# polixir/emei

Measured on AMD Instinct MI355X. Metric: env-steps/s, higher is better.
Workload: dtype f64

## Files before the change

### emei_amd/_lib.py

```python
import ctypes as C
import os

_HERE = os.path.dirname(os.path.abspath(__file__))
LIB_PATH = os.environ.get("EMEI_HIP_LIB") or os.path.join(_HERE, "libemei_hip.so")

ENV_IDS = {
    "CartPoleSwingUp": 0,
    "CartPoleBalancing": 1,
    "ReboundInvertedPendulumBalancing": 2,
    "BoundaryInvertedPendulumBalancing": 3,
    "ReboundInvertedPendulumSwingUp": 4,
    "BoundaryInvertedPendulumSwingUp": 5,
    "HalfCheetahRunning": 6,
    "ReboundInvertedDoublePendulumBalancing": 7,
    "BoundaryInvertedDoublePendulumBalancing": 8,
    "ReboundInvertedDoublePendulumSwingUp": 9,
    "BoundaryInvertedDoublePendulumSwingUp": 10,
    "HopperRunning": 11,
}
PRECISION_REF, PRECISION_F32 = 0, 1
ACT_U8, ACT_I32, ACT_I64, ACT_F32 = 0, 1, 2, 3
FLAG_AUTO_RESET = 1
DONE_TERMINAL, DONE_TRUNCATED = 1, 2
OK, ERR_INVALID, ERR_HIP, ERR_UNSUPPORTED, ERR_STATE = 0, -1, -2, -3, -4
# ... 47 lines not shown
        ("solver", C.c_uint32),
        ("env_params", C.c_double * MAX_ENV_PARAMS),
        ("ode_method", C.c_int32),
        ("rollout_chunk_steps", C.c_int32),
    ]


_vp, _i32, _i64, _u32, _u64, _dbl = C.c_void_p, C.c_int32, C.c_int64, C.c_uint32, C.c_uint64, C.c_double
SYMBOLS = {
    "emei_create": (C.c_int, [C.POINTER(EmeiConfig), C.POINTER(_vp)]),
    "emei_destroy": (C.c_int, [_vp]),
    "emei_last_error": (C.c_char_p, []),
    "emei_abi_version": (C.c_int, []),
    "emei_model_constants": (C.c_int, [C.c_int, _vp, C.c_int]),
    "emei_model_invweights": (C.c_int, [C.c_int, _vp, C.c_int]),
    "emei_env_dims": (C.c_int, [C.c_int, C.POINTER(C.c_int), C.POINTER(C.c_int), C.POINTER(C.c_int)]),
    "emei_reset": (C.c_int, [_vp, _u64, _vp]),
    "emei_set_seed": (C.c_int, [_vp, _u64]),
    "emei_get_solver_cap_hits": (C.c_int, [_vp, _vp, _vp]),
    "emei_get_rollout_faults": (C.c_int, [_vp, _vp, _vp]),
    "emei_last_rollout_kernel": (C.c_int, [_vp]),
    "emei_set_obs_peers": (C.c_int, [_vp, C.c_int, C.POINTER(_vp), _i64, _i64, _i32]),
    "emei_peer_buffer_create": (C.c_int, [C.c_int, _u64, C.POINTER(_vp), _vp]),
    "emei_peer_buffer_open": (C.c_int, [C.c_int, _vp, C.POINTER(_vp)]),
    "emei_peer_buffer_close": (C.c_int, [C.c_int, _vp]),
    "emei_peer_buffer_destroy": (C.c_int, [C.c_int, _vp]),
    "emei_set_state": (C.c_int, [_vp, _vp, C.c_int, _vp]),
    "emei_get_state": (C.c_int, [_vp, _vp, _vp]),
    "emei_get_obs": (C.c_int, [_vp, _vp, _vp]),
    "emei_freeze": (C.c_int, [_vp, _vp]),
# ... 82 lines not shown
```

### emei_amd/csrc/abi.hip

```cpp
#include <hip/hip_runtime.h>

#include <cmath>
#include <cstdarg>
#include <cstdio>
#include <cstring>
#include <ctime>
#include <new>

#include "launch.h"
#include "body_kernels.h"
#include "cheetah_model.h"
#include "hopper_model.h"
#include "dpend_model.h"

using namespace emei;

struct emei_env {
    emei_config cfg;
    int obs_dim, act_dim, state_dim;
    size_t real_size;
    void* state;
    int32_t* steps;
    uint32_t* episode;
    unsigned long long* done_mask;
// ... 64 lines not shown
        case EMEI_IP_REBOUND_SWINGUP:
        case EMEI_IP_BOUNDARY_SWINGUP: n = ip_xml_constants(buf); break;
        case EMEI_IDP_REBOUND_BALANCING:
        case EMEI_IDP_BOUNDARY_BALANCING:
        case EMEI_IDP_REBOUND_SWINGUP:
        case EMEI_IDP_BOUNDARY_SWINGUP: n = dpend::xml_constants(buf); break;
        case EMEI_HALFCHEETAH_RUNNING: n = cheetah::xml_constants(buf); break;
        case EMEI_HOPPER_RUNNING: n = hopper::xml_constants(buf); break;
        case EMEI_CARTPOLE_SWINGUP:
        case EMEI_CARTPOLE_BALANCING: return fail(EMEI_ERR_UNSUPPORTED, "emei_model_constants: CartPole has no model file (cartpole.py:22-27)");
        default: return fail(EMEI_ERR_INVALID, "unknown env_id %d", env_id);
    }
    if (n > capacity) return fail(EMEI_ERR_INVALID, "emei_model_constants: %d values, capacity %d", n, capacity);
    memcpy(out, buf, n * sizeof(double));
    return n;
}

extern "C" EMEI_API int emei_model_invweights(int env_id, double* out, int capacity) {
    if (!out || capacity < 0) return fail(EMEI_ERR_INVALID, "emei_model_invweights: bad argument");
    double buf[32];
    int n;
    switch (env_id) {
        case EMEI_IP_REBOUND_BALANCING:
        case EMEI_IP_BOUNDARY_BALANCING:
        case EMEI_IP_REBOUND_SWINGUP:
        case EMEI_IP_BOUNDARY_SWINGUP: {
            constexpr IpModel m = ip_make_model(false);
            buf[0] = m.invw, buf[1] = m.invw_hinge, n = 2;
            break;
        }
// ... 1158 lines not shown
```

### emei_amd/csrc/body_kernels.h

```cpp
#pragma once
#include "emei_device.h"
#include "launch.h"

namespace emei {

struct EnvParams {
    uint32_t mask = 0;
    double v[EMEI_MAX_ENV_PARAMS] = {0};
    double get(int k, double dflt) const { return (mask >> k) & 1u ? v[k] : dflt; }
};

struct NoiseSpec {
    float init[EMEI_MAX_STATE_DIM] = {0}, obs[EMEI_MAX_STATE_DIM] = {0};
    int32_t shared = 0;
};
template <int NS>
struct NoiseArgs {
    float init[NS], obs[NS];
    int32_t shared, obs_on;
    NoiseArgs() = default;
    explicit NoiseArgs(const NoiseSpec& h) : shared(h.shared), obs_on(0) {
        for (int i = 0; i < NS; ++i) init[i] = h.init[i], obs[i] = h.obs[i], obs_on |= h.obs[i] != 0.f;
    }
};
// ... 19 lines not shown
        boxmuller(r.v[0], r.v[1], z[4 * b], z[4 * b + 1]);
        boxmuller(r.v[2], r.v[3], z[4 * b + 2], z[4 * b + 3]);
    }
#pragma unroll
    for (int i = 0; i < NS; ++i) {
        const R d = (R)__fmul_rn(sig[i], z[i]);
        s[i] = ASSIGN ? d : s[i] + d;
    }
}
template <class Body>
__device__ __forceinline__ void body_init(typename Body::real (&s)[Body::NS], uint64_t seed, uint64_t env, uint32_t episode,
                                          const NoiseArgs<Body::NS>& ns) {
    gauss_state<typename Body::real, Body::NS, true>(s, seed, env, episode, 0u, ns.init, ns.shared != 0);
    Body::init_base(s);
}

template <class Body, bool RK4>
__device__ __forceinline__ void body_substep(typename Body::real (&s)[Body::NS], const typename Body::real (&ctrl)[Body::NA],
                                             const typename Body::Model& m, bool semi, const TrigCtx& trig,
                                             typename Body::Warm& warm) {
    using R = typename Body::real;
    constexpr int NV = Body::NS / 2;
    const R dt = (R)m.dt;
    R q[NV], v[NV], acc[NV];
#pragma unroll
    for (int i = 0; i < NV; ++i) q[i] = s[i], v[i] = s[NV + i];
    if constexpr (!RK4) {
        typename Body::Warm cold{};
        Body::accel(q, v, ctrl, m, dt, acc, trig, cold);
#pragma unroll
// ... 161 lines not shown
    constexpr int kWaves = kBlock / kWave;
    constexpr int kActVec = (kWave * NA + 3) / 4, kObsVec = (kWave * NO + 3) / 4;
    constexpr int kActIt = (kActVec + kWave - 1) / kWave, kObsIt = (kObsVec + kWave - 1) / kWave;
    __shared__ __attribute__((aligned(16))) float act_s[kWaves][kActIt * kWave * 4];
    __shared__ __attribute__((aligned(16))) float obs_s[kWaves][kObsIt * kWave * 4];
    __shared__ SinCosEntry trig_s[kTrigTableSize];
    stage_trig_table<kBlock>(trig_s, a.trig);
    TrigCtx trig;
    trig.tab = trig_s;
    __shared__ R scratch_s[(Body::kScratchPerLane > 0 ? Body::kScratchPerLane : 1) * (Body::kScratchPerLane > 0 ? kBlock : 1)];
    if constexpr (Body::kScratchPerLane > 0) trig.scratch = scratch_s;
    trig.scratch_stride = kBlock;
    trig.cap_hits = a.cap_hits;
    EMEI_PROFILE_BEGIN();
    const int lane = threadIdx.x & (kWave - 1), wv = threadIdx.x / kWave;
    constexpr bool kQueue = QUEUE;
    uint32_t ticket = 0;
    [[maybe_unused]] bool first_item = true;
    if constexpr (kQueue) {
        if (lane == 0) ticket = __hip_atomic_fetch_add(a.work + WorkQueue::kTicket, 1u, __ATOMIC_RELAXED, __HIP_MEMORY_SCOPE_AGENT);
    }
#pragma nounroll
    for (;;) {
    EMEI_CLOCK_BEGIN();
    uint32_t blk = blockIdx.x, chunk = 0;
    int t_begin = 0, t_end = a.n_steps;
    if constexpr (kQueue) {
        ticket = __builtin_amdgcn_readfirstlane(ticket);
        if (ticket >= a.n_items) {
            EMEI_CLOCK_WORKER_EXIT();
// ... 78 lines not shown
        } else {
#pragma unroll
            for (int c = 0; c < kActIt; ++c) ((float4*)act_s[wv])[c * kWave + lane] = av[c];
            wave_lds_fence();
#pragma unroll
            for (int k = 0; k < NA; ++k) ctrl[k] = (R)act_s[wv][lane * NA + k];
            wave_lds_fence();
            if (t + 1 < t_end) fetch_actions(t + 1);
        }

        R pre[NS];
#pragma unroll
        for (int k = 0; k < NS; ++k) pre[k] = s[k];
        typename Body::Warm warm{};
        for (int k = 0; k < a.freq_rate; ++k) {
            body_substep<Body, RK4>(s, ctrl, a.m, a.semi != 0, trig, warm);
            if (obs_noise)
                gauss_state<R, NS, false>(s, a.seed ^ kObsNoiseKey, a.env_offset + (uint64_t)i, episode,
                                          ((uint32_t)steps * (uint32_t)a.freq_rate + (uint32_t)k) * (uint32_t)((NS + 3) / 4),
                                          a.noise.obs, a.noise.shared != 0);
        }
        EMEI_MARK(step_io);
        float o[NO];
        R rew;
        bool term;
        Body::outputs(s, pre, ctrl, a.m, a.freq_rate, o, rew, term, trig);
        ++steps;
        const bool trunc = (a.max_episode_steps > 0) & (steps >= a.max_episode_steps);
        done = active ? ((term ? EMEI_DONE_TERMINAL : 0u) | (trunc ? EMEI_DONE_TRUNCATED : 0u)) : 0u;

        if (a.obs_out) {
            float* mine = &obs_s[wv][lane * NO];
#pragma unroll
            for (int k = 0; k < NO; ++k) mine[k] = o[k];
            wave_lds_fence();
            float* dst = a.obs_out + ((int64_t)t * n + i0) * NO;
            if (wave_envs == kWave && (((uintptr_t)dst) & 15u) == 0) {
#pragma unroll
                for (int c = 0; c < kObsIt; ++c) {
                    const int vec = c * kWave + lane;
                    if (vec < kObsVec) store_body_out<Body::kStreamOutputs>((float4*)dst + vec, ((const float4*)obs_s[wv])[vec]);
// ... 133 lines not shown
        __syncthreads();
    }
    if (threadIdx.x == 0) *out = part[0];
}
template <class Body, typename T>
__global__ void __launch_bounds__(kBlock)
    body_terminal_kernel(const T* obs, uint8_t* terminal, int64_t n, typename Body::Model m) {
    const int64_t i = (int64_t)blockIdx.x * kBlock + threadIdx.x;
    if (i >= n) return;
    terminal[i] = (uint8_t)Body::batch_terminal(obs + i * Body::NO, m);
}

template <class Body, bool RK4, typename T>
__global__ void __launch_bounds__(kBlock)
    body_next_obs_kernel(const T* obs, const float* actions, T* next_obs, int64_t n, int freq_rate, int semi,
                         typename Body::Model m, const SinCosEntry* trig_tab) {
    using R = typename Body::real;
    constexpr int NS = Body::NS, NO = Body::NO, NA = Body::NA;
    static_assert(NS == NO, "observation and state must have the same layout");
    __shared__ SinCosEntry trig_s[kTrigTableSize];
    stage_trig_table(trig_s, trig_tab);
    TrigCtx trig;
    trig.tab = trig_s;
    __shared__ R scratch_s[(Body::kScratchPerLane > 0 ? Body::kScratchPerLane : 1) * (Body::kScratchPerLane > 0 ? kBlock : 1)];
    if constexpr (Body::kScratchPerLane > 0) trig.scratch = scratch_s;
    const int64_t i = (int64_t)blockIdx.x * kBlock + threadIdx.x;
    if (i >= n) return;
    R s[NS], pre[NS], ctrl[NA], rew;
#pragma unroll
    for (int k = 0; k < NS; ++k) s[k] = pre[k] = (R)obs[i * NO + k];
#pragma unroll
    for (int k = 0; k < NA; ++k) ctrl[k] = (R)actions[i * NA + k];
    typename Body::Warm warm{};
    for (int k = 0; k < freq_rate; ++k) body_substep<Body, RK4>(s, ctrl, m, semi != 0, trig, warm);
    if constexpr (sizeof(T) == 8) {
        double o[NO];
        Body::obs_of(s, o, m);
#pragma unroll
        for (int k = 0; k < NO; ++k) next_obs[i * NO + k] = o[k];
    } else {
        float o[NO];
        bool term;
        Body::outputs(s, pre, ctrl, m, freq_rate, o, rew, term, trig);
#pragma unroll
        for (int k = 0; k < NO; ++k) next_obs[i * NO + k] = o[k];
    }
}

template <class Body, bool RK4, bool DRAWN = false, bool KEEP = false, class Spec = CandidateSpec>
__global__ void __launch_bounds__(kBlock)
    body_plan_kernel(const typename Body::real* state, const double* start_rows, const float* actions, int64_t n_envs,
                     int32_t n_cand, int32_t horizon, double discount, int freq_rate, int semi, typename Body::Model m,
                     const SinCosEntry* trig_tab, unsigned long long* cap_hits, double* ret_out, int32_t* len_out, float* final_obs,
                     Spec sp, PlanPartial* partials) {
    using R = typename Body::real;
    constexpr int NS = Body::NS, NO = Body::NO, NA = Body::NA;
    __shared__ SinCosEntry trig_s[kTrigTableSize];
    stage_trig_table(trig_s, trig_tab);
    TrigCtx trig;
    trig.tab = trig_s;
    __shared__ R scratch_s[(Body::kScratchPerLane > 0 ? Body::kScratchPerLane : 1) * (Body::kScratchPerLane > 0 ? kBlock : 1)];
    if constexpr (Body::kScratchPerLane > 0) trig.scratch = scratch_s;
    trig.scratch_stride = kBlock;
    trig.cap_hits = cap_hits;
    const int64_t nk = n_envs * n_cand;
    const int64_t j = (int64_t)blockIdx.x * kBlock + threadIdx.x;
    const bool active = j < nk;
    const int64_t i = (active ? j : 0) / n_cand;
    R s[NS], parked[NS];
    if (start_rows) {
#pragma unroll
        for (int k = 0; k < NS; ++k) s[k] = (R)start_rows[i * NS + k];
    } else {
#pragma unroll
        for (int k = 0; k < NS; ++k) s[k] = state[(int64_t)k * n_envs + i];
    }
    Body::park(parked);
#pragma unroll
    for (int k = 0; k < NS; ++k) s[k] = active ? s[k] : parked[k];
// ... 230 lines not shown
```

### emei_amd/csrc/body_mpc_kernels.h

```cpp
#pragma once

namespace emei {

template <class Body>
struct BodyMpcArgs {
    typename Body::real* state;
    int32_t* steps;
    uint32_t* episode;
    const SinCosEntry* trig;
    unsigned long long* cap_hits;
    float* nominal;
    double* work;
    float* actions_out;
    float* obs_out;
    float* reward_out;
    uint8_t* done_out;
    double* plan_return_out;
    double* ess_out;
    double* elite_return_out;
    int64_t n;
    int32_t n_steps, horizon, n_cand, n_elites, iterations, freq_rate, max_episode_steps, semi;
    uint32_t flags;
    uint64_t reset_seed, env_offset, seed;
    double discount, temperature;
    float sigma, sigma_min, lo, hi, refill, nominal_lo, nominal_hi;
    NoiseArgs<Body::NS> noise;
    typename Body::Model m;
};

template <class Body, bool RK4, class Spec>
__device__ __forceinline__ void body_mpc_score(const typename Body::real (&s)[Body::NS], const Spec& sp, uint64_t g, int lane,
                                               const BodyMpcArgs<Body>& a, const TrigCtx& trig, double* wt, double& rs, int32_t& ks) {
    using R = typename Body::real;
    constexpr int NS = Body::NS, NO = Body::NO, NA = Body::NA;
    rs = __builtin_nan("");
    ks = INT32_MAX;
    for (int32_t k0 = 0; k0 < a.n_cand; k0 += kWave) {
        const int32_t k = k0 + lane;
        R cs[NS];
#pragma unroll
        for (int q = 0; q < NS; ++q) cs[q] = s[q];
        double ret = 0.0, gd = 1.0;
        bool live = k < a.n_cand;
        for (int32_t h = 0; h < a.horizon; ++h) {
            R ctrl[NA];
            CandidateWords cw(sp.seed, g, (uint32_t)k);
#pragma unroll
            for (int q = 0; q < NA; ++q) ctrl[q] = (R)draw_action(cw, sp, 1, 0, h, q, NA);
            R pre[NS];
#pragma unroll
            for (int q = 0; q < NS; ++q) pre[q] = cs[q];
            typename Body::Warm warm{};
            for (int f = 0; f < a.freq_rate; ++f) body_substep<Body, RK4>(cs, ctrl, a.m, a.semi != 0, trig, warm);
            float o[NO];
            R rew;
            bool term;
            Body::outputs(cs, pre, ctrl, a.m, a.freq_rate, o, rew, term, trig);
            if (live) {
                ret = ret + gd * (double)(float)rew;
                gd = gd * a.discount;
                if (term) live = false;
            }
            if (__ballot(live) == 0ull) break;
        }
        if (k < a.n_cand) {
            wt[k] = ret;
            if (plan_replaces(rs, ks, ret, k)) rs = ret, ks = k;
        }
    }
#pragma unroll
    for (int d = 1; d < kWave; d <<= 1) {
        const double r2 = __shfl_xor(rs, d, kWave);
        const int32_t k2 = __shfl_xor(ks, d, kWave);
        if (plan_replaces(rs, ks, r2, k2)) rs = r2, ks = k2;
    }
}

template <class Body, bool RK4>
__device__ __forceinline__ uint32_t body_mpc_act_step(typename Body::real (&s)[Body::NS], int32_t& steps, uint32_t& episode, float* nom,
                                                      int32_t n_comp, int32_t t, int64_t i, uint64_t g, int lane,
                                                      const BodyMpcArgs<Body>& a, const TrigCtx& trig) {
    using R = typename Body::real;
    constexpr int NS = Body::NS, NO = Body::NO, NA = Body::NA;
    const int64_t at = (int64_t)t * a.n + i;
    R ctrl[NA];
#pragma unroll
    for (int q = 0; q < NA; ++q) {
        const float av = nom[q];
        ctrl[q] = (R)av;
        if (lane == 0) a.actions_out[at * NA + q] = av;
    }
    R pre[NS];
#pragma unroll
    for (int q = 0; q < NS; ++q) pre[q] = s[q];
    typename Body::Warm warm{};
    for (int f = 0; f < a.freq_rate; ++f) body_substep<Body, RK4>(s, ctrl, a.m, a.semi != 0, trig, warm);
    float o[NO];
    R rew;
    bool term;
    Body::outputs(s, pre, ctrl, a.m, a.freq_rate, o, rew, term, trig);
    ++steps;
    const bool trunc = (a.max_episode_steps > 0) & (steps >= a.max_episode_steps);
    const uint32_t done = (term ? EMEI_DONE_TERMINAL : 0u) | (trunc ? EMEI_DONE_TRUNCATED : 0u);
    if (lane == 0) {
        if (a.obs_out) {
#pragma unroll
            for (int q = 0; q < NO; ++q) a.obs_out[at * NO + q] = o[q];
        }
        if (a.reward_out) a.reward_out[at] = (float)rew;
        if (a.done_out) a.done_out[at] = (uint8_t)done;
    }
    const bool reset_now = (a.flags & EMEI_FLAG_AUTO_RESET) != 0 && __builtin_amdgcn_readfirstlane(done) != 0u;
    if (reset_now) {
        ++episode;
        steps = 0;
// ... 25 lines not shown
}

template <class Body, bool RK4>
__global__ void __launch_bounds__(kBlock) body_mpc_mppi_kernel(const BodyMpcArgs<Body> a) {
    static_assert(Body::kFusedMpc && Body::kScratchPerLane == 0, "a body without block scratch that opted in");
    using R = typename Body::real;
    constexpr int kWavesPerBlock = kBlock / kWave;
    constexpr int NS = Body::NS, na = Body::NA;
    __shared__ SinCosEntry trig_s[kTrigTableSize];
    __shared__ float nom_s[kWavesPerBlock][EMEI_MPC_MAX_HORIZON * na];
    stage_trig_table(trig_s, a.trig);
    TrigCtx trig;
    trig.tab = trig_s;
    trig.scratch_stride = kBlock;
    trig.cap_hits = a.cap_hits;
    const int lane = (int)(threadIdx.x & (kWave - 1));
    const int wv = __builtin_amdgcn_readfirstlane((int)(threadIdx.x / kWave));
    const int64_t i = (int64_t)blockIdx.x * kWavesPerBlock + wv;
    if (i >= a.n) return;
    const int64_t n = a.n;
    const int32_t n_cand = a.n_cand;
    const int32_t n_comp = a.horizon * na;
    float* nom = nom_s[wv];
    for (int32_t c = lane; c < n_comp; c += kWave) nom[c] = a.nominal[((int64_t)(c / na) * n + i) * na + c % na];

    R s[NS];
#pragma unroll
    for (int k = 0; k < NS; ++k) s[k] = a.state[(int64_t)k * n + i];
    int32_t steps = a.steps[i];
    uint32_t episode = a.episode[i];
    const uint64_t g = a.env_offset + (uint64_t)i;
    double* wt = a.work + i * n_cand;
    CandidateSpecLds sp;
    sp.env_offset = a.env_offset;
    sp.nominal.p = (const __attribute__((address_space(3))) float*)nom;
    sp.sigma = a.sigma, sp.lo = a.lo, sp.hi = a.hi;
    uint32_t done = 0;

    for (int32_t t = 0; t < a.n_steps; ++t) {
        for (int32_t cc = lane; cc < n_comp; cc += kWave) nom[cc] = fminf(fmaxf(nom[cc], a.nominal_lo), a.nominal_hi);
        wave_lds_fence();
        sp.seed = a.seed + (uint64_t)t;
        double rs;
        int32_t ks;
        body_mpc_score<Body, RK4>(s, sp, g, lane, a, trig, wt, rs, ks);
        double z = 0.0, z2 = 0.0;
        for (int32_t k = lane; k < n_cand; k += kWave) {
            const double r = wt[k];
            const double e = exp((r - rs) / a.temperature);
            const double w = rs != rs ? 1.0 : (r != r ? 0.0 : (r == rs ? 1.0 : e));
            wt[k] = w;
            z += w, z2 += w * w;
        }
#pragma unroll
        for (int d = 1; d < kWave; d <<= 1) z += __shfl_xor(z, d, kWave);
#pragma unroll
        for (int d = 1; d < kWave; d <<= 1) z2 += __shfl_xor(z2, d, kWave);
        if (lane == 0) {
            if (a.plan_return_out) a.plan_return_out[(int64_t)t * n + i] = rs;
            if (a.ess_out) a.ess_out[(int64_t)t * n + i] = z * z / z2;
// ... 13 lines not shown
#pragma unroll
            for (int u = 0; u < 4; ++u) {
#pragma unroll
                for (int d = 1; d < kWave; d <<= 1) acc[u] += __shfl_xor(acc[u], d, kWave);
            }
            wave_lds_fence();
            if (lane == 0) {
#pragma unroll
                for (int u = 0; u < 4; ++u) {
                    const int32_t cc = c0 + u;
                    if (cc < n_comp) nom[cc] = (float)(acc[u] / z);
                }
            }
        }
        wave_lds_fence();
        done = body_mpc_act_step<Body, RK4>(s, steps, episode, nom, n_comp, t, i, g, lane, a, trig);
    }
    body_mpc_write_back<Body>(s, steps, episode, done, nom, n_comp, i, lane, wt, a);
}

template <class Body, bool RK4>
__global__ void __launch_bounds__(kBlock) body_mpc_cem_kernel(const BodyMpcArgs<Body> a) {
    static_assert(Body::kFusedMpc && Body::kScratchPerLane == 0, "a body without block scratch that opted in");
    using R = typename Body::real;
    constexpr int kWavesPerBlock = kBlock / kWave;
    constexpr int NS = Body::NS, na = Body::NA;
    __shared__ SinCosEntry trig_s[kTrigTableSize];
    __shared__ float nom_s[kWavesPerBlock][EMEI_MPC_MAX_HORIZON * na];
    __shared__ float sig_s[kWavesPerBlock][EMEI_MPC_MAX_HORIZON * na];
    __shared__ uint32_t hist_s[kWavesPerBlock][256];
    stage_trig_table(trig_s, a.trig);
    TrigCtx trig;
    trig.tab = trig_s;
    trig.scratch_stride = kBlock;
    trig.cap_hits = a.cap_hits;
    const int lane = (int)(threadIdx.x & (kWave - 1));
    const int wv = __builtin_amdgcn_readfirstlane((int)(threadIdx.x / kWave));
    const int64_t i = (int64_t)blockIdx.x * kWavesPerBlock + wv;
    if (i >= a.n) return;
    const int64_t n = a.n;
    const int32_t n_cand = a.n_cand;
    const int32_t n_comp = a.horizon * na;
    float* nom = nom_s[wv];
    float* sig = sig_s[wv];
    uint32_t* hist = hist_s[wv];
    for (int32_t c = lane; c < n_comp; c += kWave) nom[c] = a.nominal[((int64_t)(c / na) * n + i) * na + c % na];

    R s[NS];
#pragma unroll
    for (int k = 0; k < NS; ++k) s[k] = a.state[(int64_t)k * n + i];
// ... 7 lines not shown
    sp.sigma_map.p = (const __attribute__((address_space(3))) float*)sig;
    sp.lo = a.lo, sp.hi = a.hi;
    const double m_el = (double)a.n_elites;
    uint32_t done = 0;

    for (int32_t t = 0; t < a.n_steps; ++t) {
        for (int32_t it = 0; it < a.iterations; ++it) {
            for (int32_t cc = lane; cc < n_comp; cc += kWave) {
                nom[cc] = fminf(fmaxf(nom[cc], a.nominal_lo), a.nominal_hi);
                if (it == 0) sig[cc] = a.sigma;
            }
            wave_lds_fence();
            sp.seed = a.seed + (uint64_t)t * (uint64_t)a.iterations + (uint64_t)it;
            double rs;
            int32_t ks;
            body_mpc_score<Body, RK4>(s, sp, g, lane, a, trig, wt, rs, ks);
            const bool last_it = it == a.iterations - 1;
            if (lane == 0 && last_it && a.plan_return_out) a.plan_return_out[(int64_t)t * n + i] = rs;
            uint64_t prefix = 0ull;
            int32_t need = a.n_elites;
            for (int shift = 56; shift >= 0; shift -= 8) {
#pragma unroll
                for (int b = 0; b < 4; ++b) hist[4 * lane + b] = 0u;
                wave_lds_fence();
                for (int32_t k = lane; k < n_cand; k += kWave) {
                    const uint64_t key = plan_key(wt[k]);
                    const uint64_t high = shift == 56 ? 0ull : key >> (shift + 8);
                    if (high == prefix) atomicAdd(&hist[(uint32_t)(key >> shift) & 255u], 1u);
                }
                wave_lds_fence();
                int32_t cb[4], own = 0;
// ... 63 lines not shown
                if (lane == 0) {
#pragma unroll
                    for (int u = 0; u < 4; ++u) {
                        const int32_t cc = c0 + u;
                        if (cc >= n_comp) continue;
                        const double mu = s1[u] / m_el;
                        nom[cc] = (float)(m0[u] + mu);
                        sig[cc] = (float)sqrt(fmax(s2[u] / m_el - mu * mu, 0.0));
                    }
                }
            }
            wave_lds_fence();
            for (int32_t cc = lane; cc < n_comp; cc += kWave) sig[cc] = fmaxf(sig[cc], a.sigma_min);
            wave_lds_fence();
        }
        done = body_mpc_act_step<Body, RK4>(s, steps, episode, nom, n_comp, t, i, g, lane, a, trig);
    }
    body_mpc_write_back<Body>(s, steps, episode, done, nom, n_comp, i, lane, wt, a);
}

template <class Body>
static int launch_body_mpc(const BodyLaunch& L, const typename Body::Model& m) {
    const MpcLaunch& M = L.mpc;
    const bool cem = L.op == BODY_OP_MPC_CEM;
    if (M.horizon < 1 || M.horizon > EMEI_MPC_MAX_HORIZON) return EMEI_ERR_INVALID;
    if (cem && (M.iterations < 1 || M.n_elites < 1 || M.n_elites > L.plan.n_candidates)) return EMEI_ERR_INVALID;
    if (NoiseArgs<Body::NS>(L.noise).obs_on) return EMEI_ERR_UNSUPPORTED;
    BodyMpcArgs<Body> a;
    a.state = (typename Body::real*)L.state, a.steps = L.steps, a.episode = L.episode;
    a.trig = (const SinCosEntry*)L.trig, a.cap_hits = L.cap_hits;
    a.nominal = M.nominal, a.work = L.plan.return_out, a.actions_out = M.actions_out;
// ... 26 lines not shown
```

### emei_amd/csrc/dpend_model.h

```cpp
#pragma once
#include <cmath>
#include <cstring>

#include "emei_device.h"

namespace emei {
namespace dpend {

struct Model {
    double s1z, s2z, diag1, diag2, L1, mtot;
    double gx, gz, gear, x_lo, x_hi, margin, invw;
    double K, B, dmin, dmax, width;
    double dt, phi_off;
};

namespace host {
inline double capsule_mass(double rho, double r, double half) { return rho * (M_PI * r * r * 2 * half + 4.0 / 3.0 * M_PI * r * r * r); }
inline double capsule_inertia_perp(double rho, double r, double half) {
    double h = 2 * half, mcyl = rho * M_PI * r * r * h, msph = rho * 4.0 / 3.0 * M_PI * r * r * r;
    return mcyl * (3 * r * r + h * h) / 12 + msph * (2 * r * r / 5 + h * h / 4 + 3 * h * r / 8);
}
}

struct Xml {
    double rho, cart_r, cart_half, pole_r, pole_half, L1, gx, gz, gear, ctrl_lo, ctrl_hi, x_lo, x_hi, margin, solref_tc, dmin, dmax, width;
};
constexpr Xml kXml = {1000.0, 0.1, 0.1,
                      0.045, 0.3, 0.6,
                      1e-5, 9.81,
                      500.0, -1.0, 1.0,
                      -3.0, 3.0, 0.01,
                      0.02, 0.9, 0.95, 0.001};

inline Model make_model(bool swingup, double dt) {
    Model m;
    memset(&m, 0, sizeof(m));
    const double rho = kXml.rho;
    const double mc = host::capsule_mass(rho, kXml.cart_r, kXml.cart_half);
    const double mp = host::capsule_mass(rho, kXml.pole_r, kXml.pole_half);
    const double Ip = host::capsule_inertia_perp(rho, kXml.pole_r, kXml.pole_half);
    const double lc = kXml.pole_half, L1 = kXml.L1;
    m.s1z = mp * lc + mp * L1, m.s2z = mp * lc;
    m.diag1 = Ip + mp * lc * lc + mp * L1 * L1, m.diag2 = Ip + mp * lc * lc;
    m.L1 = L1, m.mtot = mc + 2 * mp;
    m.gx = kXml.gx, m.gz = kXml.gz;
    m.gear = kXml.gear;
    m.x_lo = kXml.x_lo, m.x_hi = kXml.x_hi, m.margin = kXml.margin;
    const double a = m.mtot, b = m.s1z, c = m.s2z, d = m.diag1, e = L1 * m.s2z, f = m.diag2;
    const double det = a * (d * f - e * e) - b * (b * f - e * c) + c * (b * e - d * c);
    m.invw = (d * f - e * e) / det;
    const double tc = kXml.solref_tc < 2 * dt ? 2 * dt : kXml.solref_tc, dmax = kXml.dmax;
    m.K = 1.0 / (dmax * dmax * tc * tc), m.B = 2.0 / (dmax * tc);
    m.dmin = kXml.dmin, m.dmax = dmax, m.width = kXml.width;
    m.dt = dt;
    m.phi_off = swingup ? M_PI : 0.0;
    return m;
}

inline int xml_constants(double* out) {
    const double mc = host::capsule_mass(kXml.rho, kXml.cart_r, kXml.cart_half), mp = host::capsule_mass(kXml.rho, kXml.pole_r, kXml.pole_half);
    const double v[17] = {kXml.gx, kXml.gz, mc, mp, host::capsule_inertia_perp(kXml.rho, kXml.pole_r, kXml.pole_half), kXml.pole_half,
                          kXml.L1, kXml.gear, kXml.ctrl_lo, kXml.ctrl_hi, kXml.x_lo, kXml.x_hi, kXml.margin, kXml.solref_tc, kXml.dmin,
                          kXml.dmax, kXml.width};
    for (int i = 0; i < 17; ++i) out[i] = v[i];
    return 17;
}

}

template <int VARIANT, typename R>
struct DPendBody {
    using real = R;
    using Model = dpend::Model;
    static constexpr int kMinWavesPerEU = 1;
    static constexpr bool kUnrollRK4 = false;
    static constexpr int kScratchPerLane = 0;
    static constexpr bool kFusedMpc = true;
    static constexpr bool kHasCtrlCost = false;
    static constexpr bool kObsIsState = false;
    static constexpr bool kSpareReset = true;
    static constexpr bool kStreamOutputs = true;
    static constexpr int NS = 6, NO = 6, NA = 1;
    static Model make_model(double dt, const EnvParams&) { return dpend::make_model(VARIANT >= 2, dt); }

    struct Warm {};
    __device__ __forceinline__ static void begin_stages(Warm&) {}
    __device__ __forceinline__ static void accel(const R (&q)[3], const R (&v)[3], const R (&ctrl)[NA], const Model& m, R,
                                                 R (&qacc)[3], const TrigCtx& trig, Warm&) {
        const R phi1 = q[1] + (R)m.phi_off, phi2 = phi1 + q[2];
        const R w1 = v[1], w2 = v[1] + v[2];
        R s1, c1, s2, c2;
        sincos_ctx(trig, phi1, s1, c1);
        sincos_ctx(trig, phi2, s2, c2);
        const R S1x = (R)m.s1z * s1, S1z = (R)m.s1z * c1, S2x = (R)m.s2z * s2, S2z = (R)m.s2z * c2;
        const R Dx = (R)m.L1 * s1, Dz = (R)m.L1 * c1;
        const R M12 = fma_r(Dx, S2x, Dz * S2z);
        const R u = ctrl[0] < R(dpend::kXml.ctrl_lo) ? R(dpend::kXml.ctrl_lo) : (ctrl[0] > R(dpend::kXml.ctrl_hi) ? R(dpend::kXml.ctrl_hi) : ctrl[0]);
        const R w1s = w1 * w1, w2s = w2 * w2;
        R fx = (R)m.gear * u + (R)m.mtot * (R)m.gx + w1s * S1x + w2s * S2x;
        R f1 = (R)m.gx * S1z + (R)m.gz * S1x + w2s * fma_r(S2x, Dz, -(S2z * Dx));
        R f2 = (R)m.gx * S2z + (R)m.gz * S2x + w1s * fma_r(Dx, S2z, -(Dz * S2x));
        const R a = (R)m.mtot, b = S1z, c = S2z, d = (R)m.diag1, e = M12, f = (R)m.diag2;
        const R if_ = rcp1_r(f);
        const R le = e * if_, lc = c * if_;
        const R d1 = fma_r(-le, e, d), b1 = fma_r(-le, c, b), a1 = fma_r(-lc, c, a);
        const R id1 = rcp1_r(d1);
        const R lb = b1 * id1;
        const R a2 = fma_r(-lb, b1, a1);
        const R ia2 = rcp1_r(a2);
        R ax, a1_, a2_;
        {
            const R y1 = fma_r(-le, f2, f1);
            const R yx = fma_r(-lb, y1, fma_r(-lc, f2, fx));
            ax = yx * ia2;
            a1_ = fma_r(-lb, ax, y1 * id1);
            a2_ = fma_r(-le, a1_, fma_r(-lc, ax, f2 * if_));
        }
        static_assert(dpend::kXml.x_lo == -dpend::kXml.x_hi, "symmetric slider range");
        const R ax_abs = abs_r(q[0]);
        if (ax_abs > (R)(m.x_hi - m.margin)) {
            const R nJ = copysign_r(R(1), q[0]);
            const R n1 = fma_r((R)m.B, v[0], ax);
            const R wx = ia2, w1_ = -lb * ia2, w2_ = fma_r(lb, le, -lc) * ia2;
            auto finish = [&](R Kimp, R Kimp_edge, R Rr) __attribute__((always_inline)) {
                const R num = fma_r(nJ, n1, fma_r(Kimp, ax_abs, -Kimp_edge));
                const R g = nJ * fmax_r(num * rcp1_r(wx + Rr), R(0));
                ax = fma_r(-wx, g, ax);
                a1_ = fma_r(-w1_, g, a1_);
                a2_ = fma_r(-w2_, g, a2_);
            };
            const R edge = (R)(m.x_hi - m.margin);
            const R Kfull = (R)m.K * (R)m.dmax;
            const bool full = !(ax_abs < (R)(m.x_hi - m.margin + m.width));
            if (__builtin_expect(__ballot(!full) != 0ull, 0)) {
                const R xx = (ax_abs - edge) * (R)(1.0 / m.width), u1 = R(1) - xx;
                const R y = xx <= R(0.5) ? R(2) * xx * xx : fma_r(R(-2) * u1, u1, R(1));
                const R imp = fma_r(y, (R)(m.dmax - m.dmin), (R)m.dmin);
                const R Kimp = full ? Kfull : (R)m.K * imp;
                finish(Kimp, Kimp * edge, full ? (R)((1.0 - m.dmax) / m.dmax) * (R)m.invw : (R(1) - imp) * (R)m.invw * rcp1_r(imp));
            } else {
                finish(Kfull, Kfull * edge, (R)((1.0 - m.dmax) / m.dmax) * (R)m.invw);
            }
        }
        qacc[0] = ax, qacc[1] = a1_, qacc[2] = a2_ - a1_;
    }

    template <typename T>
    __device__ __forceinline__ static T quirk_wrap(T th) {
        const T pi = T(3.141592653589793);
        return pymod_pos(th + pi, T(2), T(0.5)) * pi - pi;
    }
    template <typename T, typename SC>
    __device__ __forceinline__ static void reward_terminal(const T (&o)[NO], const Model& m, T& rew, bool& term, SC sc) {
        T sa, ca, sb, cb;
        sc(o[1], sa, ca);
        sc(o[1] + o[2], sb, cb);
        const T y = ca + cb;
        bool fin = true;
#pragma unroll
        for (int k = 0; k < NO; ++k) fin &= finite_r(o[k]);
        const bool inx = ((T)m.x_lo < o[0]) & (o[0] < (T)m.x_hi);
        if (VARIANT == 0) rew = T(1), term = !((y >= T(1.5)) & fin);
        else if (VARIANT == 1) rew = T(1), term = !((y >= T(0)) & inx & fin);
        else if (VARIANT == 2) rew = (T(2) - y) / T(4), term = !fin;
        else rew = (T(2) - y) / T(4) - (T(5e-3) * o[4] * o[4] + T(1e-4) * o[5] * o[5]), term = !(inx & fin);
    }
    __device__ __forceinline__ static void outputs(const R (&s)[NS], const R (&pre)[NS], const R (&ctrl)[NA], const Model& m,
                                                   int freq_rate, float (&o)[NO], R& rew, bool& term, const TrigCtx& trig) {
        R ob[NO] = {s[0], quirk_wrap(s[1]), quirk_wrap(s[2]), s[3], s[4], s[5]};
        reward_terminal(ob, m, rew, term, [&](R x, R& sn, R& cs) { sincos_ctx(trig, x, sn, cs); });
#pragma unroll
        for (int k = 0; k < NO; ++k) o[k] = (float)ob[k];
    }
    __device__ __forceinline__ static void init_base(R (&)[NS]) {}
    __device__ __forceinline__ static void park(R (&s)[NS]) {
#pragma unroll
// ... 28 lines not shown
```

### include/emei_hip.h

```cpp
#ifndef EMEI_HIP_H
#define EMEI_HIP_H

#include <stdint.h>

#ifdef __cplusplus
extern "C" {
#endif

#define EMEI_ABI_VERSION 8

#if defined(__GNUC__)
#define EMEI_API __attribute__((visibility("default")))
#else
#define EMEI_API
#endif

enum emei_env_id {
    EMEI_CARTPOLE_SWINGUP = 0,
    EMEI_CARTPOLE_BALANCING = 1,
    EMEI_IP_REBOUND_BALANCING = 2,
    EMEI_IP_BOUNDARY_BALANCING = 3,
    EMEI_IP_REBOUND_SWINGUP = 4,
    EMEI_IP_BOUNDARY_SWINGUP = 5,
    EMEI_HALFCHEETAH_RUNNING = 6,
// ... 64 lines not shown
    uint32_t solver;
    double env_params[EMEI_MAX_ENV_PARAMS];
    int32_t ode_method;
    int32_t rollout_chunk_steps;
} emei_config;
#define EMEI_CONFIG_SIZE_V1 64u

EMEI_API int emei_create(const emei_config* cfg, emei_env** out);
EMEI_API int emei_destroy(emei_env* h);
EMEI_API const char* emei_last_error(void);
EMEI_API int emei_abi_version(void);

EMEI_API int emei_model_constants(int env_id, double* out, int capacity);

EMEI_API int emei_model_invweights(int env_id, double* out, int capacity);

EMEI_API int emei_env_dims(int env_id, int* obs_dim, int* act_dim, int* state_dim);

EMEI_API int emei_reset(emei_env* h, uint64_t seed, void* stream);

EMEI_API int emei_set_state(emei_env* h, const double* state_aos, int reset_counters, void* stream);
EMEI_API int emei_get_state(emei_env* h, double* state_aos, void* stream);
EMEI_API int emei_get_obs(emei_env* h, double* obs_aos, void* stream);

EMEI_API int emei_freeze(emei_env* h, void* stream);
EMEI_API int emei_unfreeze(emei_env* h, void* stream);

EMEI_API int emei_get_solver_cap_hits(emei_env* h, uint64_t* count_out, void* stream);

EMEI_API int emei_get_rollout_faults(emei_env* h, uint64_t* count_out, void* stream);
// ... 123 lines not shown
```

Before: 279.0 billion.

## Make double-pendulum model constants compile-time and hoist diag2 reciprocal per thread

Splits the double-pendulum model into constexpr geometry constants and runtime parameters (dt, K, B). The kernels now fold the constants at compile time instead of loading them from the kernel argument struct. The reciprocal of diag2 is computed once per thread through a new device_model hook rather than in every accel call. A host ABI function is added to export the model values. Constant folding shrinks kernel arguments and arithmetic, with some added template complexity.

```diff
diff --git a/emei_amd/_lib.py b/emei_amd/_lib.py
--- a/emei_amd/_lib.py
+++ b/emei_amd/_lib.py
@@ -85,6 +85,7 @@
     "emei_abi_version": (C.c_int, []),
     "emei_model_constants": (C.c_int, [C.c_int, _vp, C.c_int]),
     "emei_model_invweights": (C.c_int, [C.c_int, _vp, C.c_int]),
+    "emei_dpend_model_values": (C.c_int, [C.c_int, C.c_double, _vp, C.c_int]),
     "emei_env_dims": (C.c_int, [C.c_int, C.POINTER(C.c_int), C.POINTER(C.c_int), C.POINTER(C.c_int)]),
     "emei_reset": (C.c_int, [_vp, _u64, _vp]),
     "emei_set_seed": (C.c_int, [_vp, _u64]),
diff --git a/emei_amd/csrc/abi.hip b/emei_amd/csrc/abi.hip
--- a/emei_amd/csrc/abi.hip
+++ b/emei_amd/csrc/abi.hip
@@ -102,6 +102,11 @@
     if (n > capacity) return fail(EMEI_ERR_INVALID, "emei_model_constants: %d values, capacity %d", n, capacity);
     memcpy(out, buf, n * sizeof(double));
     return n;
+}
+
+extern "C" EMEI_API int emei_dpend_model_values(int swingup, double dt, double* out, int capacity) {
+    if (!out || capacity < 20) return fail(EMEI_ERR_INVALID, "emei_dpend_model_values: bad argument");
+    return swingup ? dpend::model_values<true>(dt, out) : dpend::model_values<false>(dt, out);
 }
 
 extern "C" EMEI_API int emei_model_invweights(int env_id, double* out, int capacity) {
diff --git a/emei_amd/csrc/body_kernels.h b/emei_amd/csrc/body_kernels.h
--- a/emei_amd/csrc/body_kernels.h
+++ b/emei_amd/csrc/body_kernels.h
@@ -57,6 +57,15 @@
     gauss_state<typename Body::real, Body::NS, true>(s, seed, env, episode, 0u, ns.init, ns.shared != 0);
     Body::init_base(s);
 }
+
+template <class Body, class = void>
+struct body_model_of {
+    __device__ __forceinline__ static const typename Body::Model& get(const typename Body::Model& m) { return m; }
+};
+template <class Body>
+struct body_model_of<Body, decltype((void)&Body::device_model)> {
+    __device__ __forceinline__ static typename Body::Model get(const typename Body::Model& m) { return Body::device_model(m); }
+};
 
 template <class Body, bool RK4>
 __device__ __forceinline__ void body_substep(typename Body::real (&s)[Body::NS], const typename Body::real (&ctrl)[Body::NA],
@@ -248,6 +257,7 @@
     trig.cap_hits = a.cap_hits;
     EMEI_PROFILE_BEGIN();
     const int lane = threadIdx.x & (kWave - 1), wv = threadIdx.x / kWave;
+    decltype(auto) m = body_model_of<Body>::get(a.m);
     constexpr bool kQueue = QUEUE;
     uint32_t ticket = 0;
     [[maybe_unused]] bool first_item = true;
@@ -356,7 +366,7 @@
         for (int k = 0; k < NS; ++k) pre[k] = s[k];
         typename Body::Warm warm{};
         for (int k = 0; k < a.freq_rate; ++k) {
-            body_substep<Body, RK4>(s, ctrl, a.m, a.semi != 0, trig, warm);
+            body_substep<Body, RK4>(s, ctrl, m, a.semi != 0, trig, warm);
             if (obs_noise)
                 gauss_state<R, NS, false>(s, a.seed ^ kObsNoiseKey, a.env_offset + (uint64_t)i, episode,
                                           ((uint32_t)steps * (uint32_t)a.freq_rate + (uint32_t)k) * (uint32_t)((NS + 3) / 4),
@@ -366,7 +376,7 @@
         float o[NO];
         R rew;
         bool term;
-        Body::outputs(s, pre, ctrl, a.m, a.freq_rate, o, rew, term, trig);
+        Body::outputs(s, pre, ctrl, m, a.freq_rate, o, rew, term, trig);
         ++steps;
         const bool trunc = (a.max_episode_steps > 0) & (steps >= a.max_episode_steps);
         done = active ? ((term ? EMEI_DONE_TERMINAL : 0u) | (trunc ? EMEI_DONE_TRUNCATED : 0u)) : 0u;
@@ -530,7 +540,7 @@
 template <class Body, bool RK4, typename T>
 __global__ void __launch_bounds__(kBlock)
     body_next_obs_kernel(const T* obs, const float* actions, T* next_obs, int64_t n, int freq_rate, int semi,
-                         typename Body::Model m, const SinCosEntry* trig_tab) {
+                         typename Body::Model m_arg, const SinCosEntry* trig_tab) {
     using R = typename Body::real;
     constexpr int NS = Body::NS, NO = Body::NO, NA = Body::NA;
     static_assert(NS == NO, "observation and state must have the same layout");
@@ -542,6 +552,7 @@
     if constexpr (Body::kScratchPerLane > 0) trig.scratch = scratch_s;
     const int64_t i = (int64_t)blockIdx.x * kBlock + threadIdx.x;
     if (i >= n) return;
+    decltype(auto) m = body_model_of<Body>::get(m_arg);
     R s[NS], pre[NS], ctrl[NA], rew;
 #pragma unroll
     for (int k = 0; k < NS; ++k) s[k] = pre[k] = (R)obs[i * NO + k];
@@ -566,7 +577,7 @@
 template <class Body, bool RK4, bool DRAWN = false, bool KEEP = false, class Spec = CandidateSpec>
 __global__ void __launch_bounds__(kBlock)
     body_plan_kernel(const typename Body::real* state, const double* start_rows, const float* actions, int64_t n_envs,
-                     int32_t n_cand, int32_t horizon, double discount, int freq_rate, int semi, typename Body::Model m,
+                     int32_t n_cand, int32_t horizon, double discount, int freq_rate, int semi, typename Body::Model m_arg,
                      const SinCosEntry* trig_tab, unsigned long long* cap_hits, double* ret_out, int32_t* len_out, float* final_obs,
                      Spec sp, PlanPartial* partials) {
     using R = typename Body::real;
@@ -579,6 +590,7 @@
     if constexpr (Body::kScratchPerLane > 0) trig.scratch = scratch_s;
     trig.scratch_stride = kBlock;
     trig.cap_hits = cap_hits;
+    decltype(auto) m = body_model_of<Body>::get(m_arg);
     const int64_t nk = n_envs * n_cand;
     const int64_t j = (int64_t)blockIdx.x * kBlock + threadIdx.x;
     const bool active = j < nk;
diff --git a/emei_amd/csrc/body_mpc_kernels.h b/emei_amd/csrc/body_mpc_kernels.h
--- a/emei_amd/csrc/body_mpc_kernels.h
+++ b/emei_amd/csrc/body_mpc_kernels.h
@@ -30,7 +30,8 @@
 
 template <class Body, bool RK4, class Spec>
 __device__ __forceinline__ void body_mpc_score(const typename Body::real (&s)[Body::NS], const Spec& sp, uint64_t g, int lane,
-                                               const BodyMpcArgs<Body>& a, const TrigCtx& trig, double* wt, double& rs, int32_t& ks) {
+                                               const BodyMpcArgs<Body>& a, const typename Body::Model& m, const TrigCtx& trig, double* wt,
+                                               double& rs, int32_t& ks) {
     using R = typename Body::real;
     constexpr int NS = Body::NS, NO = Body::NO, NA = Body::NA;
     rs = __builtin_nan("");
@@ -51,11 +52,11 @@
 #pragma unroll
             for (int q = 0; q < NS; ++q) pre[q] = cs[q];
             typename Body::Warm warm{};
-            for (int f = 0; f < a.freq_rate; ++f) body_substep<Body, RK4>(cs, ctrl, a.m, a.semi != 0, trig, warm);
+            for (int f = 0; f < a.freq_rate; ++f) body_substep<Body, RK4>(cs, ctrl, m, a.semi != 0, trig, warm);
             float o[NO];
             R rew;
             bool term;
-            Body::outputs(cs, pre, ctrl, a.m, a.freq_rate, o, rew, term, trig);
+            Body::outputs(cs, pre, ctrl, m, a.freq_rate, o, rew, term, trig);
             if (live) {
                 ret = ret + gd * (double)(float)rew;
                 gd = gd * a.discount;
@@ -79,7 +80,7 @@
 template <class Body, bool RK4>
 __device__ __forceinline__ uint32_t body_mpc_act_step(typename Body::real (&s)[Body::NS], int32_t& steps, uint32_t& episode, float* nom,
                                                       int32_t n_comp, int32_t t, int64_t i, uint64_t g, int lane,
-                                                      const BodyMpcArgs<Body>& a, const TrigCtx& trig) {
+                                                      const BodyMpcArgs<Body>& a, const typename Body::Model& m, const TrigCtx& trig) {
     using R = typename Body::real;
     constexpr int NS = Body::NS, NO = Body::NO, NA = Body::NA;
     const int64_t at = (int64_t)t * a.n + i;
@@ -94,11 +95,11 @@
 #pragma unroll
     for (int q = 0; q < NS; ++q) pre[q] = s[q];
     typename Body::Warm warm{};
-    for (int f = 0; f < a.freq_rate; ++f) body_substep<Body, RK4>(s, ctrl, a.m, a.semi != 0, trig, warm);
+    for (int f = 0; f < a.freq_rate; ++f) body_substep<Body, RK4>(s, ctrl, m, a.semi != 0, trig, warm);
     float o[NO];
     R rew;
     bool term;
-    Body::outputs(s, pre, ctrl, a.m, a.freq_rate, o, rew, term, trig);
+    Body::outputs(s, pre, ctrl, m, a.freq_rate, o, rew, term, trig);
     ++steps;
     const bool trunc = (a.max_episode_steps > 0) & (steps >= a.max_episode_steps);
     const uint32_t done = (term ? EMEI_DONE_TERMINAL : 0u) | (trunc ? EMEI_DONE_TRUNCATED : 0u);
@@ -154,6 +155,7 @@
     trig.tab = trig_s;
     trig.scratch_stride = kBlock;
     trig.cap_hits = a.cap_hits;
+    decltype(auto) m = body_model_of<Body>::get(a.m);
     const int lane = (int)(threadIdx.x & (kWave - 1));
     const int wv = __builtin_amdgcn_readfirstlane((int)(threadIdx.x / kWave));
     const int64_t i = (int64_t)blockIdx.x * kWavesPerBlock + wv;
@@ -183,7 +185,7 @@
         sp.seed = a.seed + (uint64_t)t;
         double rs;
         int32_t ks;
-        body_mpc_score<Body, RK4>(s, sp, g, lane, a, trig, wt, rs, ks);
+        body_mpc_score<Body, RK4>(s, sp, g, lane, a, m, trig, wt, rs, ks);
         double z = 0.0, z2 = 0.0;
         for (int32_t k = lane; k < n_cand; k += kWave) {
             const double r = wt[k];
@@ -227,7 +229,7 @@
             }
         }
         wave_lds_fence();
-        done = body_mpc_act_step<Body, RK4>(s, steps, episode, nom, n_comp, t, i, g, lane, a, trig);
+        done = body_mpc_act_step<Body, RK4>(s, steps, episode, nom, n_comp, t, i, g, lane, a, m, trig);
     }
     body_mpc_write_back<Body>(s, steps, episode, done, nom, n_comp, i, lane, wt, a);
 }
@@ -247,6 +249,7 @@
     trig.tab = trig_s;
     trig.scratch_stride = kBlock;
     trig.cap_hits = a.cap_hits;
+    decltype(auto) m = body_model_of<Body>::get(a.m);
     const int lane = (int)(threadIdx.x & (kWave - 1));
     const int wv = __builtin_amdgcn_readfirstlane((int)(threadIdx.x / kWave));
     const int64_t i = (int64_t)blockIdx.x * kWavesPerBlock + wv;
@@ -284,7 +287,7 @@
             sp.seed = a.seed + (uint64_t)t * (uint64_t)a.iterations + (uint64_t)it;
             double rs;
             int32_t ks;
-            body_mpc_score<Body, RK4>(s, sp, g, lane, a, trig, wt, rs, ks);
+            body_mpc_score<Body, RK4>(s, sp, g, lane, a, m, trig, wt, rs, ks);
             const bool last_it = it == a.iterations - 1;
             if (lane == 0 && last_it && a.plan_return_out) a.plan_return_out[(int64_t)t * n + i] = rs;
             uint64_t prefix = 0ull;
@@ -378,7 +381,7 @@
             for (int32_t cc = lane; cc < n_comp; cc += kWave) sig[cc] = fmaxf(sig[cc], a.sigma_min);
             wave_lds_fence();
         }
-        done = body_mpc_act_step<Body, RK4>(s, steps, episode, nom, n_comp, t, i, g, lane, a, trig);
+        done = body_mpc_act_step<Body, RK4>(s, steps, episode, nom, n_comp, t, i, g, lane, a, m, trig);
     }
     body_mpc_write_back<Body>(s, steps, episode, done, nom, n_comp, i, lane, wt, a);
 }
diff --git a/emei_amd/csrc/dpend_model.h b/emei_amd/csrc/dpend_model.h
--- a/emei_amd/csrc/dpend_model.h
+++ b/emei_amd/csrc/dpend_model.h
@@ -7,16 +7,20 @@
 namespace emei {
 namespace dpend {
 
-struct Model {
+struct Consts {
     double s1z, s2z, diag1, diag2, L1, mtot;
     double gx, gz, gear, x_lo, x_hi, margin, invw;
-    double K, B, dmin, dmax, width;
-    double dt, phi_off;
-};
+    double dmin, dmax, width;
+    double phi_off;
+};
+struct Params {
+    double dt, K, B;
+};
+struct Model : Consts, Params {};
 
 namespace host {
-inline double capsule_mass(double rho, double r, double half) { return rho * (M_PI * r * r * 2 * half + 4.0 / 3.0 * M_PI * r * r * r); }
-inline double capsule_inertia_perp(double rho, double r, double half) {
+constexpr double capsule_mass(double rho, double r, double half) { return rho * (M_PI * r * r * 2 * half + 4.0 / 3.0 * M_PI * r * r * r); }
+constexpr double capsule_inertia_perp(double rho, double r, double half) {
     double h = 2 * half, mcyl = rho * M_PI * r * r * h, msph = rho * 4.0 / 3.0 * M_PI * r * r * r;
     return mcyl * (3 * r * r + h * h) / 12 + msph * (2 * r * r / 5 + h * h / 4 + 3 * h * r / 8);
 }
@@ -32,9 +36,8 @@
                       -3.0, 3.0, 0.01,
                       0.02, 0.9, 0.95, 0.001};
 
-inline Model make_model(bool swingup, double dt) {
-    Model m;
-    memset(&m, 0, sizeof(m));
+constexpr Consts make_consts(bool swingup) {
+    Consts m{};
     const double rho = kXml.rho;
     const double mc = host::capsule_mass(rho, kXml.cart_r, kXml.cart_half);
     const double mp = host::capsule_mass(rho, kXml.pole_r, kXml.pole_half);
@@ -49,12 +52,31 @@
     const double a = m.mtot, b = m.s1z, c = m.s2z, d = m.diag1, e = L1 * m.s2z, f = m.diag2;
     const double det = a * (d * f - e * e) - b * (b * f - e * c) + c * (b * e - d * c);
     m.invw = (d * f - e * e) / det;
-    const double tc = kXml.solref_tc < 2 * dt ? 2 * dt : kXml.solref_tc, dmax = kXml.dmax;
-    m.K = 1.0 / (dmax * dmax * tc * tc), m.B = 2.0 / (dmax * tc);
-    m.dmin = kXml.dmin, m.dmax = dmax, m.width = kXml.width;
-    m.dt = dt;
+    m.dmin = kXml.dmin, m.dmax = kXml.dmax, m.width = kXml.width;
     m.phi_off = swingup ? M_PI : 0.0;
     return m;
+}
+constexpr Params make_params(double dt) {
+    Params p{};
+    const double tc = kXml.solref_tc < 2 * dt ? 2 * dt : kXml.solref_tc, dmax = kXml.dmax;
+    p.K = 1.0 / (dmax * dmax * tc * tc), p.B = 2.0 / (dmax * tc);
+    p.dt = dt;
+    return p;
+}
+inline Model make_model(bool swingup, double dt) {
+    Model m;
+    static_cast<Consts&>(m) = make_consts(swingup);
+    static_cast<Params&>(m) = make_params(dt);
+    return m;
+}
+template <bool SWINGUP>
+inline int model_values(double dt, double* out) {
+    constexpr Consts c = make_consts(SWINGUP);
+    const Params p = make_params(dt);
+    const double v[20] = {c.s1z, c.s2z, c.diag1, c.diag2, c.L1, c.mtot, c.gx, c.gz, c.gear, c.x_lo, c.x_hi, c.margin, c.invw,
+                          c.dmin, c.dmax, c.width, c.phi_off, p.dt, p.K, p.B};
+    for (int i = 0; i < 20; ++i) out[i] = v[i];
+    return 20;
 }
 
 inline int xml_constants(double* out) {
@@ -71,7 +93,10 @@
 template <int VARIANT, typename R>
 struct DPendBody {
     using real = R;
-    using Model = dpend::Model;
+    struct Model {
+        double dt, K, B;
+        R if2;
+    };
     static constexpr int kMinWavesPerEU = 1;
     static constexpr bool kUnrollRK4 = false;
     static constexpr int kScratchPerLane = 0;
@@ -81,27 +106,39 @@
     static constexpr bool kSpareReset = true;
     static constexpr bool kStreamOutputs = true;
     static constexpr int NS = 6, NO = 6, NA = 1;
-    static Model make_model(double dt, const EnvParams&) { return dpend::make_model(VARIANT >= 2, dt); }
+    static Model make_model(double dt, const EnvParams&) {
+        const dpend::Params p = dpend::make_params(dt);
+        return Model{p.dt, p.K, p.B, R(0)};
+    }
+    __device__ __forceinline__ static Model device_model(const Model& arg) {
+        constexpr dpend::Consts kc = dpend::make_consts(VARIANT >= 2);
+        R f = (R)kc.diag2;
+        asm volatile("" : "+v"(f));
+        Model m = arg;
+        m.if2 = rcp1_r(f);
+        return m;
+    }
 
     struct Warm {};
     __device__ __forceinline__ static void begin_stages(Warm&) {}
     __device__ __forceinline__ static void accel(const R (&q)[3], const R (&v)[3], const R (&ctrl)[NA], const Model& m, R,
                                                  R (&qacc)[3], const TrigCtx& trig, Warm&) {
-        const R phi1 = q[1] + (R)m.phi_off, phi2 = phi1 + q[2];
+        constexpr dpend::Consts kc = dpend::make_consts(VARIANT >= 2);
+        const R phi1 = q[1] + (R)kc.phi_off, phi2 = phi1 + q[2];
         const R w1 = v[1], w2 = v[1] + v[2];
         R s1, c1, s2, c2;
         sincos_ctx(trig, phi1, s1, c1);
         sincos_ctx(trig, phi2, s2, c2);
-        const R S1x = (R)m.s1z * s1, S1z = (R)m.s1z * c1, S2x = (R)m.s2z * s2, S2z = (R)m.s2z * c2;
-        const R Dx = (R)m.L1 * s1, Dz = (R)m.L1 * c1;
+        const R S1x = (R)kc.s1z * s1, S1z = (R)kc.s1z * c1, S2x = (R)kc.s2z * s2, S2z = (R)kc.s2z * c2;
+        const R Dx = (R)kc.L1 * s1, Dz = (R)kc.L1 * c1;
         const R M12 = fma_r(Dx, S2x, Dz * S2z);
         const R u = ctrl[0] < R(dpend::kXml.ctrl_lo) ? R(dpend::kXml.ctrl_lo) : (ctrl[0] > R(dpend::kXml.ctrl_hi) ? R(dpend::kXml.ctrl_hi) : ctrl[0]);
         const R w1s = w1 * w1, w2s = w2 * w2;
-        R fx = (R)m.gear * u + (R)m.mtot * (R)m.gx + w1s * S1x + w2s * S2x;
-        R f1 = (R)m.gx * S1z + (R)m.gz * S1x + w2s * fma_r(S2x, Dz, -(S2z * Dx));
-        R f2 = (R)m.gx * S2z + (R)m.gz * S2x + w1s * fma_r(Dx, S2z, -(Dz * S2x));
-        const R a = (R)m.mtot, b = S1z, c = S2z, d = (R)m.diag1, e = M12, f = (R)m.diag2;
-        const R if_ = rcp1_r(f);
+        R fx = (R)kc.gear * u + (R)kc.mtot * (R)kc.gx + w1s * S1x + w2s * S2x;
+        R f1 = (R)kc.gx * S1z + (R)kc.gz * S1x + w2s * fma_r(S2x, Dz, -(S2z * Dx));
+        R f2 = (R)kc.gx * S2z + (R)kc.gz * S2x + w1s * fma_r(Dx, S2z, -(Dz * S2x));
+        const R a = (R)kc.mtot, b = S1z, c = S2z, d = (R)kc.diag1, e = M12;
+        const R if_ = m.if2;
         const R le = e * if_, lc = c * if_;
         const R d1 = fma_r(-le, e, d), b1 = fma_r(-le, c, b), a1 = fma_r(-lc, c, a);
         const R id1 = rcp1_r(d1);
@@ -118,7 +155,7 @@
         }
         static_assert(dpend::kXml.x_lo == -dpend::kXml.x_hi, "symmetric slider range");
         const R ax_abs = abs_r(q[0]);
-        if (ax_abs > (R)(m.x_hi - m.margin)) {
+        if (ax_abs > (R)(kc.x_hi - kc.margin)) {
             const R nJ = copysign_r(R(1), q[0]);
             const R n1 = fma_r((R)m.B, v[0], ax);
             const R wx = ia2, w1_ = -lb * ia2, w2_ = fma_r(lb, le, -lc) * ia2;
@@ -129,17 +166,17 @@
                 a1_ = fma_r(-w1_, g, a1_);
                 a2_ = fma_r(-w2_, g, a2_);
             };
-            const R edge = (R)(m.x_hi - m.margin);
-            const R Kfull = (R)m.K * (R)m.dmax;
-            const bool full = !(ax_abs < (R)(m.x_hi - m.margin + m.width));
+            const R edge = (R)(kc.x_hi - kc.margin);
+            const R Kfull = (R)m.K * (R)kc.dmax;
+            const bool full = !(ax_abs < (R)(kc.x_hi - kc.margin + kc.width));
             if (__builtin_expect(__ballot(!full) != 0ull, 0)) {
-                const R xx = (ax_abs - edge) * (R)(1.0 / m.width), u1 = R(1) - xx;
+                const R xx = (ax_abs - edge) * (R)(1.0 / kc.width), u1 = R(1) - xx;
                 const R y = xx <= R(0.5) ? R(2) * xx * xx : fma_r(R(-2) * u1, u1, R(1));
-                const R imp = fma_r(y, (R)(m.dmax - m.dmin), (R)m.dmin);
+                const R imp = fma_r(y, (R)(kc.dmax - kc.dmin), (R)kc.dmin);
                 const R Kimp = full ? Kfull : (R)m.K * imp;
-                finish(Kimp, Kimp * edge, full ? (R)((1.0 - m.dmax) / m.dmax) * (R)m.invw : (R(1) - imp) * (R)m.invw * rcp1_r(imp));
+                finish(Kimp, Kimp * edge, full ? (R)((1.0 - kc.dmax) / kc.dmax) * (R)kc.invw : (R(1) - imp) * (R)kc.invw * rcp1_r(imp));
             } else {
-                finish(Kfull, Kfull * edge, (R)((1.0 - m.dmax) / m.dmax) * (R)m.invw);
+                finish(Kfull, Kfull * edge, (R)((1.0 - kc.dmax) / kc.dmax) * (R)kc.invw);
             }
         }
         qacc[0] = ax, qacc[1] = a1_, qacc[2] = a2_ - a1_;
@@ -152,6 +189,7 @@
     }
     template <typename T, typename SC>
     __device__ __forceinline__ static void reward_terminal(const T (&o)[NO], const Model& m, T& rew, bool& term, SC sc) {
+        constexpr dpend::Consts kc = dpend::make_consts(VARIANT >= 2);
         T sa, ca, sb, cb;
         sc(o[1], sa, ca);
         sc(o[1] + o[2], sb, cb);
@@ -159,7 +197,7 @@
         bool fin = true;
 #pragma unroll
         for (int k = 0; k < NO; ++k) fin &= finite_r(o[k]);
-        const bool inx = ((T)m.x_lo < o[0]) & (o[0] < (T)m.x_hi);
+        const bool inx = ((T)kc.x_lo < o[0]) & (o[0] < (T)kc.x_hi);
         if (VARIANT == 0) rew = T(1), term = !((y >= T(1.5)) & fin);
         else if (VARIANT == 1) rew = T(1), term = !((y >= T(0)) & inx & fin);
         else if (VARIANT == 2) rew = (T(2) - y) / T(4), term = !fin;
diff --git a/include/emei_hip.h b/include/emei_hip.h
--- a/include/emei_hip.h
+++ b/include/emei_hip.h
@@ -102,6 +102,7 @@
 EMEI_API int emei_model_constants(int env_id, double* out, int capacity);
 
 EMEI_API int emei_model_invweights(int env_id, double* out, int capacity);
+EMEI_API int emei_dpend_model_values(int swingup, double dt, double* out, int capacity);
 
 EMEI_API int emei_env_dims(int env_id, int* obs_dim, int* act_dim, int* state_dim);
 
```

Result: no change. 278.5 billion (-0.2%).
